# ChainSafe/co-zkvms

Measured on AMD Instinct MI355X. Metric: RISC-V cycles proved/sec (co-Jolt hot path: PST13 commit + dense GKR grand product + openings), higher is better.
Workload: dtype u32-limb BN254 Fr/Fq (254-bit Montgomery integers); 1 GPU; configs[1] restated (SURVEY 8d): 2^20-cycle trace per GPU, plain prover, 128 polys (64 Fr + 32 u16 + 16 u32 + 16 flags) PST13 batch commit, dense grand product 8 x 2^21 leaves, batch evaluate + opening reduction + PST13 open; log_n=20, polys=128, gp_batch=8, parallelism=single GPU, ranks_per_gpu=1

## Files before the change

co-zkvms_amd/csrc/msm.hip:

```cpp
#include "common.hpp"
#include "fq9.hip.hpp"

static constexpr uint32_t NB = 1u << 15;
static constexpr int CH = 16;
static constexpr int TPB = 256;

template <int KIND>
struct ScalarKind;
template <>
struct ScalarKind<COZK_SCALAR_FR> {
    static constexpr int NWIN = 16;
    static __device__ __forceinline__ bool load(const void* p, size_t i, uint32_t w[8]) {
        fe s = Fr::from_mont(fe_load(reinterpret_cast<const fe*>(p) + i));
#pragma unroll
        for (int k = 0; k < 8; k++) w[k] = s.l[k];
        return false;
    }
};
template <>
struct ScalarKind<COZK_SCALAR_U8> {
    static constexpr int NWIN = 1;
    static __device__ __forceinline__ bool load(const void* p, size_t i, uint32_t w[8]) {
        w[0] = reinterpret_cast<const uint8_t*>(p)[i];
        return false;
    }
};
template <>
struct ScalarKind<COZK_SCALAR_U16> {
    static constexpr int NWIN = 2;
    static __device__ __forceinline__ bool load(const void* p, size_t i, uint32_t w[8]) {
        w[0] = reinterpret_cast<const uint16_t*>(p)[i];
        return false;
    }
};
template <>
struct ScalarKind<COZK_SCALAR_U32> {
    static constexpr int NWIN = 3;
    static __device__ __forceinline__ bool load(const void* p, size_t i, uint32_t w[8]) {
        w[0] = reinterpret_cast<const uint32_t*>(p)[i];
        w[1] = 0;
        return false;
    }
};
template <>
struct ScalarKind<COZK_SCALAR_U64> {
    static constexpr int NWIN = 5;
    static __device__ __forceinline__ bool load(const void* p, size_t i, uint32_t w[8]) {
        uint64_t v = reinterpret_cast<const uint64_t*>(p)[i];
        w[0] = (uint32_t)v;
        w[1] = (uint32_t)(v >> 32);
        w[2] = 0;
        return false;
    }
};
template <>
struct ScalarKind<COZK_SCALAR_I64> {
    static constexpr int NWIN = 5;
    static __device__ __forceinline__ bool load(const void* p, size_t i, uint32_t w[8]) {
        int64_t v = reinterpret_cast<const int64_t*>(p)[i];
        bool neg = v < 0;
        uint64_t m = neg ? (uint64_t)0 - (uint64_t)v : (uint64_t)v;
        w[0] = (uint32_t)m;
        w[1] = (uint32_t)(m >> 32);
        w[2] = 0;
        return neg;
    }
};

static inline int kind_nwin(int kind) {
    switch (kind) {
        case COZK_SCALAR_FR: return 16;
        case COZK_SCALAR_U8: return 1;
        case COZK_SCALAR_U16: return 2;
        case COZK_SCALAR_U32: return 3;
        default: return 5;
    }
}

template <int KIND, class F>
__device__ __forceinline__ void for_each_digit(const void* scalars, size_t i, F&& f) {
    uint32_t w[8] = {0, 0, 0, 0, 0, 0, 0, 0};
    bool neg = ScalarKind<KIND>::load(scalars, i, w);
    uint32_t carry = 0;
#pragma unroll
    for (int k = 0; k < ScalarKind<KIND>::NWIN; k++) {
        uint32_t v = ((w[k >> 1] >> (16 * (k & 1))) & 0xffffu) + carry;
        bool sub = v > 32768u;
        carry = sub ? 1u : 0u;
        uint32_t mag = sub ? 65536u - v : v;
        f(k, mag, sub != neg);
    }
}

static __device__ __forceinline__ uint32_t agg_atomic_add(uint32_t* counters, uint32_t key, bool active) {
    uint64_t act = __ballot(active);
    uint32_t pos = 0;
    if (act == 0) return 0;
    int lane = threadIdx.x & 63;
    int first = __ffsll((unsigned long long)act) - 1;
    uint32_t k0 = __shfl(key, first);
    uint64_t same = __ballot(active && key == k0);
    int cnt = __popcll(same);
    bool merged = false;
    if (cnt >= 4) {
        uint32_t base = 0;
        if (lane == first) base = atomicAdd(&counters[k0], (uint32_t)cnt);
        base = __shfl(base, first);
        if (active && key == k0) {
            pos = base + __popcll(same & ((1ull << lane) - 1ull));
            merged = true;
        }
    }
    if (active && !merged) pos = atomicAdd(&counters[key], 1u);
    return pos;
}

template <int KIND>
__global__ void __launch_bounds__(TPB) k_msm_hist(const void* scalars, size_t n, uint32_t* hist, int grouped) {
    size_t i = (size_t)blockIdx.x * TPB + threadIdx.x;
    bool inr = i < n;
    size_t ii = inr ? i : 0;
    for_each_digit<KIND>(scalars, ii, [&](int k, uint32_t mag, bool) {
        bool act = inr && mag != 0;
        uint32_t key = (grouped ? (uint32_t)k * NB : 0u) + (mag - 1u);
        agg_atomic_add(hist, act ? key : 0u, act);
    });
}

template <int KIND>
__global__ void __launch_bounds__(TPB) k_msm_scatter(const void* scalars, size_t n, uint32_t* cursor, uint32_t* refs,
                                                  int grouped, uint32_t table_n, uint32_t base_off) {
    size_t i = (size_t)blockIdx.x * TPB + threadIdx.x;
    bool inr = i < n;
    size_t ii = inr ? i : 0;
    for_each_digit<KIND>(scalars, ii, [&](int k, uint32_t mag, bool negative) {
        bool act = inr && mag != 0;
        uint32_t key = (grouped ? (uint32_t)k * NB : 0u) + (mag - 1u);
        uint32_t pos = agg_atomic_add(cursor, act ? key : 0u, act);
        if (act) {
            uint32_t ref = (grouped ? 0u : (uint32_t)k * table_n) + base_off + (uint32_t)ii;
            refs[pos] = ref | (negative ? 0x80000000u : 0u);
        }
    });
}

struct MsmPolyDesc {
    const void* scalars;
    uint32_t n;
    uint32_t base_off;
    uint32_t group;
    uint32_t pad;
};
static constexpr int LTPB = 1024;

template <int KIND>
__global__ void __launch_bounds__(LTPB) k_msm_hist_lds(const MsmPolyDesc* __restrict__ descs, uint32_t* __restrict__ hist) {
    __shared__ uint32_t lh[NB];
    const MsmPolyDesc d = descs[blockIdx.y];
    for (uint32_t b = threadIdx.x; b < NB; b += blockDim.x) lh[b] = 0;
    __syncthreads();
    for (size_t i = (size_t)blockIdx.x * blockDim.x + threadIdx.x; i < d.n; i += (size_t)gridDim.x * blockDim.x) {
        for_each_digit<KIND>(d.scalars, i, [&](int, uint32_t mag, bool) {
            if (mag != 0) atomicAdd(&lh[mag - 1u], 1u);
        });
    }
    __syncthreads();
    uint32_t* h = hist + (size_t)d.group * NB;
    for (uint32_t b = threadIdx.x; b < NB; b += blockDim.x) {
        uint32_t c = lh[b];
        if (c) atomicAdd(&h[b], c);
    }
}

template <int KIND>
__global__ void __launch_bounds__(LTPB) k_msm_scatter_lds(const MsmPolyDesc* __restrict__ descs, uint32_t* __restrict__ cursor,
                                                       uint32_t* __restrict__ refs, uint32_t table_n) {
    __shared__ uint32_t lh[NB];
    const MsmPolyDesc d = descs[blockIdx.y];
    for (uint32_t b = threadIdx.x; b < NB; b += blockDim.x) lh[b] = 0;
    __syncthreads();
    for (size_t i = (size_t)blockIdx.x * blockDim.x + threadIdx.x; i < d.n; i += (size_t)gridDim.x * blockDim.x) {
        for_each_digit<KIND>(d.scalars, i, [&](int, uint32_t mag, bool) {
            if (mag != 0) atomicAdd(&lh[mag - 1u], 1u);
        });
    }
    __syncthreads();
    uint32_t* cur = cursor + (size_t)d.group * NB;
    for (uint32_t b = threadIdx.x; b < NB; b += blockDim.x) {
        uint32_t c = lh[b];
        lh[b] = c ? atomicAdd(&cur[b], c) : 0u;
    }
    __syncthreads();
    for (size_t i = (size_t)blockIdx.x * blockDim.x + threadIdx.x; i < d.n; i += (size_t)gridDim.x * blockDim.x) {
        for_each_digit<KIND>(d.scalars, i, [&](int k, uint32_t mag, bool negative) {
            if (mag != 0) {
                uint32_t pos = atomicAdd(&lh[mag - 1u], 1u);
                uint32_t ref = (uint32_t)k * table_n + d.base_off + (uint32_t)i;
                refs[pos] = ref | (negative ? 0x80000000u : 0u);
            }
        });
    }
}

static constexpr uint32_t SCAN_PER_BLOCK = 1024;

template <bool FROM_OFFSETS>
static __device__ __forceinline__ void scan_load4(const uint32_t* __restrict__ in, uint32_t nb, uint32_t L, uint32_t b0, uint32_t c[4],
                                                  const uint32_t* __restrict__ perm) {
#pragma unroll
    for (int k = 0; k < 4; k++) {
        uint32_t b = b0 + k;
        if (b >= nb) c[k] = 0;
        else if (FROM_OFFSETS) {
            uint32_t q = perm ? perm[b] : b;
            c[k] = (in[q + 1] - in[q] + L - 1u) / L;
        } else c[k] = in[b];
    }
}

static __device__ __forceinline__ uint32_t block_exclusive_scan_256(uint32_t v, uint32_t* sh4, uint32_t* total) {
    uint32_t x = v;
#pragma unroll
    for (int off = 1; off < 64; off <<= 1) {
        uint32_t y = __shfl_up(x, off);
        if ((int)(threadIdx.x & 63) >= off) x += y;
    }
    int w = threadIdx.x >> 6;
    if ((threadIdx.x & 63) == 63) sh4[w] = x;
    __syncthreads();
    uint32_t base = 0;
    for (int i = 0; i < w; i++) base += sh4[i];
    if (total) *total = sh4[0] + sh4[1] + sh4[2] + sh4[3];
    __syncthreads();
    return base + x - v;
}

template <bool FROM_OFFSETS>
__global__ void __launch_bounds__(256) k_scan_sums(const uint32_t* __restrict__ in, uint32_t nb, uint32_t L, uint32_t* __restrict__ bsums,
                                                 const uint32_t* __restrict__ perm) {
    __shared__ uint32_t sh4[4];
    uint32_t c[4];
    scan_load4<FROM_OFFSETS>(in, nb, L, blockIdx.x * SCAN_PER_BLOCK + threadIdx.x * 4, c, perm);
    uint32_t tot;
    (void)block_exclusive_scan_256(c[0] + c[1] + c[2] + c[3], sh4, &tot);
    if (threadIdx.x == 0) bsums[blockIdx.x] = tot;
}

__global__ void __launch_bounds__(1024) k_scan_top(uint32_t* bsums, uint32_t nblk, uint32_t* total_out) {
    __shared__ uint32_t sh[1024];
    uint32_t tid = threadIdx.x;
    uint32_t per = (nblk + 1023u) / 1024u;
    uint32_t b0 = tid * per, b1 = min(nblk, b0 + per);
    uint32_t sum = 0;
    for (uint32_t b = b0; b < b1; b++) sum += bsums[b];
    sh[tid] = sum;
    __syncthreads();
    for (uint32_t d = 1; d < 1024; d <<= 1) {
        uint32_t v = tid >= d ? sh[tid - d] : 0;
        __syncthreads();
        sh[tid] += v;
        __syncthreads();
    }
    uint32_t run = sh[tid] - sum;
    for (uint32_t b = b0; b < b1; b++) {
        uint32_t c = bsums[b];
        bsums[b] = run;
        run += c;
    }
    if (tid == 1023) *total_out = sh[1023];
}

template <bool FROM_OFFSETS>
__global__ void __launch_bounds__(256) k_scan_final(const uint32_t* in, uint32_t nb, uint32_t L, const uint32_t* __restrict__ bsums,
                                                  uint32_t* off, uint32_t* cursor, const uint32_t* __restrict__ perm) {
    __shared__ uint32_t sh4[4];
    uint32_t c[4];
    uint32_t b0 = blockIdx.x * SCAN_PER_BLOCK + threadIdx.x * 4;
    scan_load4<FROM_OFFSETS>(in, nb, L, b0, c, perm);
    uint32_t run = bsums[blockIdx.x] + block_exclusive_scan_256(c[0] + c[1] + c[2] + c[3], sh4, nullptr);
// ... 175 lines not shown
    xyzz9 acc;
    bool have = false;
    uint32_t ref_next = PF && begin < end ? refs[begin] : 0u;
    for (uint32_t e = begin; e < end; e++) {
        uint32_t ref = PF ? ref_next : refs[e];
        if (PF && e + 1 < end) ref_next = refs[e + 1];
        g1_affine p = affine_load(table + (ref & 0x7fffffffu));
        if (CHECK_INF && G1::is_inf(p)) continue;
        f9 qx = f9_from_fe(p.x), qy = f9_from_fe(p.y);
        if (ref >> 31) {
#pragma unroll
            for (int i = 0; i < 9; i++) qy.l[i] = F9_C2[i] - qy.l[i];
        }
        if (!have) {
            acc = xyzz9_from_affine(qx, qy);
            have = true;
        } else if (!madd9(acc, qx, qy)) {
            exc[1 + atomicAdd(exc, 1u)] = t;
            return;
        }
    }
    xyzz_store(out + slot, have ? xyzz9_to_xyzz(acc) : G1::identity());
}
__global__ void __launch_bounds__(TPB) k_msm_accum0_fix(const g1_affine* __restrict__ table, const uint32_t* __restrict__ refs,
                                                     const uint32_t* __restrict__ off_in, const uint32_t* __restrict__ off_out,
                                                     uint32_t nb, g1_xyzz* __restrict__ out, const uint32_t* __restrict__ exc,
                                                     const uint32_t* __restrict__ offp, const uint32_t* __restrict__ perm) {
    uint32_t n = exc[0];
    for (uint32_t q = blockIdx.x * TPB + threadIdx.x; q < n; q += gridDim.x * TPB) {
        uint32_t t = exc[1 + q];
        uint32_t begin, end, slot;
        segment_range_perm(off_in, off_out, offp, perm, nb, t, nullptr, begin, end, slot);
        xyzz_store(out + slot, gather_segment(table, refs, begin, end));
    }
}

__global__ void __launch_bounds__(TPB) k_msm_accumN(const g1_xyzz* __restrict__ in, const uint32_t* __restrict__ off_in,
                                                 const uint32_t* __restrict__ off_out, uint32_t nb, uint32_t L,
                                                 g1_xyzz* __restrict__ out, const uint32_t* __restrict__ blk) {
    uint32_t t = blockIdx.x * TPB + threadIdx.x;
    uint32_t total = off_out[nb];
    if (t >= total) return;
    uint32_t b = find_bucket_blk(off_out, nb, blk, t);
    uint32_t s = t - off_out[b];
    uint32_t cnt = off_in[b + 1] - off_in[b];
    uint32_t nseg = off_out[b + 1] - off_out[b];
    uint32_t per = (cnt + nseg - 1) / nseg;
    (void)L;
    uint32_t begin = off_in[b] + min(s * per, cnt);
    uint32_t end = off_in[b] + min((s + 1) * per, cnt);
    g1_xyzz acc = G1::identity();
    if (begin < end) acc = xyzz_load(in + begin);
    for (uint32_t e = begin + 1; e < end; e++) acc = G1::add(acc, xyzz_load(in + e));
    xyzz_store(out + t, acc);
}

static __device__ __forceinline__ g1_xyzz bucket_value(const g1_xyzz* items, const uint32_t* off, uint32_t b) {
    uint32_t o = off[b];
    if (off[b + 1] > o) return xyzz_load(items + o);
    return G1::identity();
}

__global__ void __launch_bounds__(TPB) k_msm_gather_buckets(const g1_xyzz* __restrict__ items, const uint32_t* __restrict__ off,
                                                         uint32_t nb, g1_xyzz* __restrict__ dense) {
    uint32_t b = blockIdx.x * TPB + threadIdx.x;
    if (b >= nb) return;
    xyzz_store(dense + b, bucket_value(items, off, b));
}

__global__ void __launch_bounds__(TPB) k_msm_reduce_chunks(const g1_xyzz* __restrict__ dense, uint32_t ngroups,
                                                        g1_xyzz* __restrict__ chunk_out) {
    uint32_t t = blockIdx.x * TPB + threadIdx.x;
    const uint32_t cpg = NB / CH;
    if (t >= ngroups * cpg) return;
    uint32_t g = t / cpg, c = t % cpg;
    uint32_t k0 = c * CH;
    g1_xyzz run = G1::identity(), acc = G1::identity();
    for (int j = CH - 1; j >= 0; j--) {
        run = G1::add(run, xyzz_load(dense + (size_t)g * NB + k0 + (uint32_t)j));
        acc = G1::add(acc, run);
    }
    if (c != 0 && !G1::is_identity(run)) {
        g1_xyzz m = G1::identity();
        for (int bit = 10; bit >= 0; bit--) {
            m = G1::dbl(m);
            if ((c >> bit) & 1u) m = G1::add(m, run);
        }
        for (int d = 0; d < 4; d++) m = G1::dbl(m);
        acc = G1::add(acc, m);
    }
    xyzz_store(chunk_out + t, acc);
}

__global__ void __launch_bounds__(TPB) k_msm_reduce_groups(const g1_xyzz* __restrict__ chunk, g1_xyzz* __restrict__ grp) {
    __shared__ g1_xyzz sh[TPB];
    const uint32_t cpg = NB / CH;
    uint32_t g = blockIdx.x, tid = threadIdx.x;
    g1_xyzz acc = G1::identity();
    for (uint32_t c = tid; c < cpg; c += TPB) acc = G1::add(acc, xyzz_load(chunk + (size_t)g * cpg + c));
    sh[tid] = acc;
    __syncthreads();
    for (uint32_t s = TPB / 2; s > 0; s >>= 1) {
        if (tid < s) {
            acc = G1::add(acc, sh[tid + s]);
            sh[tid] = acc;
        }
        __syncthreads();
    }
    if (tid == 0) xyzz_store(grp + g, acc);
}

__global__ void k_msm_finalize(const g1_xyzz* __restrict__ grp, uint32_t G, uint32_t npoly, g1_affine* __restrict__ out) {
    uint32_t p = blockIdx.x * blockDim.x + threadIdx.x;
    if (p >= npoly) return;
    g1_xyzz acc = xyzz_load(grp + (size_t)p * G + (G - 1));
    for (int w = (int)G - 2; w >= 0; w--) {
        for (int d = 0; d < 16; d++) acc = G1::dbl(acc);
        acc = G1::add(acc, xyzz_load(grp + (size_t)p * G + w));
    }
    affine_store(out + p, G1::to_affine(acc));
}

__global__ void __launch_bounds__(TPB) k_precompute_window(const g1_affine* __restrict__ prev, g1_affine* __restrict__ next, size_t n) {
    size_t i = (size_t)blockIdx.x * TPB + threadIdx.x;
    if (i >= n) return;
    g1_xyzz acc = G1::dbl_affine(affine_load(prev + i));
    for (int d = 1; d < 16; d++) acc = G1::dbl(acc);
    affine_store(next + i, G1::to_affine(acc));
}

__global__ void __launch_bounds__(TPB) k_fixed_base_mul(const fe* __restrict__ scalars, g1_affine g, g1_affine* __restrict__ out, size_t n) {
    size_t i = (size_t)blockIdx.x * TPB + threadIdx.x;
    if (i >= n) return;
    fe s = Fr::from_mont(fe_load(scalars + i));
    g1_xyzz acc = G1::identity();
    for (int k = 7; k >= 0; k--) {
        uint32_t w = s.l[k];
        for (int b = 31; b >= 0; b--) {
            acc = G1::dbl(acc);
            if ((w >> b) & 1u) acc = G1::add_mixed(acc, g);
        }
    }
    affine_store(out + i, G1::to_affine(acc));
}

__global__ void __launch_bounds__(TPB) k_pair_sums(const g1_affine* __restrict__ in, g1_affine* __restrict__ out, size_t nout) {
    size_t i = (size_t)blockIdx.x * TPB + threadIdx.x;
    if (i >= nout) return;
    g1_xyzz acc = G1::from_affine(affine_load(in + 2 * i));
    acc = G1::add_mixed(acc, affine_load(in + 2 * i + 1));
    affine_store(out + i, G1::to_affine(acc));
}

static inline uint32_t cdiv(uint64_t a, uint64_t b) { return (uint32_t)((a + b - 1) / b); }

__global__ void __launch_bounds__(TPB) k_any_infinity(const g1_affine* __restrict__ pts, size_t n, uint32_t* __restrict__ flag) {
    size_t i = (size_t)blockIdx.x * TPB + threadIdx.x;
    if (i < n && G1::is_inf(affine_load(pts + i))) atomicOr(flag, 1u);
}
static void build_window_table(cozk_ctx* ctx, cozk_bases* b) {
    for (int w = 1; w < b->nwin; w++) {
        k_precompute_window<<<cdiv(b->n, TPB), TPB, 0, ctx->stream>>>(b->table + (size_t)(w - 1) * b->n,
                                                                     b->table + (size_t)w * b->n, b->n);
    }
    HIP_TRY(hipGetLastError());
    ctx->scratch.reserve(64);
    uint32_t* flag = ctx->scratch.as<uint32_t>();
    HIP_TRY(hipMemsetAsync(flag, 0, 4, ctx->stream));
    k_any_infinity<<<cdiv(b->n, TPB), TPB, 0, ctx->stream>>>(b->table, b->n, flag);
    uint32_t h = 1;
    HIP_TRY(hipMemcpyAsync(&h, flag, 4, hipMemcpyDeviceToHost, ctx->stream));
    HIP_TRY(hipStreamSynchronize(ctx->stream));
    b->has_inf = h != 0;
}

#define KIND_DISPATCH(kind, CALL)                                              \
    switch (kind) {                                                            \
        case COZK_SCALAR_FR: { constexpr int K = COZK_SCALAR_FR; CALL; } break;   \
        case COZK_SCALAR_U8: { constexpr int K = COZK_SCALAR_U8; CALL; } break;   \
        case COZK_SCALAR_U16: { constexpr int K = COZK_SCALAR_U16; CALL; } break; \
        case COZK_SCALAR_U32: { constexpr int K = COZK_SCALAR_U32; CALL; } break; \
        case COZK_SCALAR_U64: { constexpr int K = COZK_SCALAR_U64; CALL; } break; \
        case COZK_SCALAR_I64: { constexpr int K = COZK_SCALAR_I64; CALL; } break; \
        default: throw CozkError(COZK_ERR_INVALID_ARG, "unknown scalar kind");    \
    }

struct MsmSetPlan {
    uint32_t P = 0, G = 1, nb = 0, L0 = 8;
    uint64_t M = 0, bound = 0, maxseg0 = 0;
    bool pre = false;
};

static MsmSetPlan msm_plan(const cozk_bases* bases, const size_t* offsets, const size_t* ns, const int* kinds, size_t P) {
    COZK_REQUIRE(P >= 1, "msm: empty batch");
    COZK_REQUIRE((uint64_t)bases->n * (uint64_t)bases->nwin < (1ull << 31), "msm: table too large for 31-bit refs");
    MsmSetPlan pl;
    pl.P = (uint32_t)P;
    pl.pre = bases->nwin == 16;
    pl.G = pl.pre ? 1u : 16u;
    pl.nb = (uint32_t)P * pl.G * NB;
    for (size_t p = 0; p < P; p++) {
        COZK_REQUIRE(offsets[p] + ns[p] <= bases->n, "msm: base slice out of range");
        uint64_t m = (uint64_t)ns[p] * kind_nwin(kinds[p]);
        pl.M += m;
        if (m > pl.bound) pl.bound = m;
    }
    COZK_REQUIRE(pl.M < (1ull << 32), "msm: batch too large (reference count exceeds 32 bits)");
    uint32_t L0 = (uint32_t)(pl.M >> 18);
    if (L0 < 8) L0 = 8;
    if (L0 > 127) L0 = 127;
    pl.L0 = L0;
    pl.maxseg0 = pl.M / L0 + pl.nb;
    return pl;
}

static void msm_scan(hipStream_t st, uint32_t* bsums, uint32_t nb, bool from_offsets, const uint32_t* in, uint32_t L, uint32_t* off, uint32_t* cursor,
                     const uint32_t* perm = nullptr) {
    const uint32_t nscan_blocks = (nb + SCAN_PER_BLOCK - 1) / SCAN_PER_BLOCK;
    if (from_offsets) {
        k_scan_sums<true><<<nscan_blocks, 256, 0, st>>>(in, nb, L, bsums, perm);
        k_scan_top<<<1, 1024, 0, st>>>(bsums, nscan_blocks, off + nb);
        k_scan_final<true><<<nscan_blocks, 256, 0, st>>>(in, nb, L, bsums, off, cursor, perm);
    } else {
        k_scan_sums<false><<<nscan_blocks, 256, 0, st>>>(in, nb, L, bsums, nullptr);
        k_scan_top<<<1, 1024, 0, st>>>(bsums, nscan_blocks, off + nb);
        k_scan_final<false><<<nscan_blocks, 256, 0, st>>>(in, nb, L, bsums, off, cursor, nullptr);
    }
}

static void msm_sort(cozk_ctx* ctx, hipStream_t st, MsmSortWs& sw, const MsmSetPlan& pl, const cozk_bases* bases, const size_t* offsets,
                     const size_t* ns, const void* const* scalars, const int* kinds) {
    const uint32_t nb = pl.nb, G = pl.G;
    const size_t P = pl.P;
    sw.hist.reserve((size_t)(nb + 2) * 4);
    sw.off0.reserve((size_t)(nb + 1) * 4);
    sw.offA.reserve((size_t)(nb + 1) * 4);
    sw.refs.reserve((size_t)pl.M * 4);
    uint32_t* hist = sw.hist.as<uint32_t>();
    uint32_t* off0 = sw.off0.as<uint32_t>();
    uint32_t* refs = sw.refs.as<uint32_t>();
    const uint32_t nscan_blocks = (nb + SCAN_PER_BLOCK - 1) / SCAN_PER_BLOCK;
    sw.ptrs.reserve((size_t)nscan_blocks * 4 + P * sizeof(MsmPolyDesc) + 64);
    uint32_t* bsums = sw.ptrs.as<uint32_t>();
    MsmPolyDesc* d_descs = reinterpret_cast<MsmPolyDesc*>(((uintptr_t)(bsums + nscan_blocks) + 15) & ~(uintptr_t)15);
    HIP_TRY(hipMemsetAsync(hist, 0, (size_t)(nb + 2) * 4, st));
    uint32_t* d_maxcnt = hist + nb + 1;
    if (!sw.max_pinned) HIP_TRY(hipHostMalloc((void**)&sw.max_pinned, 64 + 64 * sizeof(MsmPolyDesc), hipHostMallocDefault));
    if (!sw.max_event) HIP_TRY(hipEventCreateWithFlags(&sw.max_event, hipEventDisableTiming));
    auto read_back_max = [&] {
        k_max_u32<<<std::min<uint32_t>(cdiv(nb, 256), 1024u), 256, 0, st>>>(hist, nb, d_maxcnt);
        HIP_TRY(hipMemcpyAsync(sw.max_pinned, d_maxcnt, 4, hipMemcpyDeviceToHost, st));
        HIP_TRY(hipEventRecord(sw.max_event, st));
    };
    if (pl.pre) {
        MsmPolyDesc* h_descs = reinterpret_cast<MsmPolyDesc*>(reinterpret_cast<char*>(sw.max_pinned) + 64);
        COZK_REQUIRE(P <= 64, "msm: too many polynomials in one launch set");
        uint32_t nd = 0;
        std::vector<std::pair<int, std::pair<uint32_t, uint32_t>>> runs;
        size_t max_n = 0;
        for (int kind = 0; kind <= COZK_SCALAR_I64; kind++) {
            uint32_t first = nd;
            for (size_t p = 0; p < P; p++)
                if (kinds[p] == kind && ns[p]) {
                    h_descs[nd++] = MsmPolyDesc{scalars[p], (uint32_t)ns[p], (uint32_t)offsets[p], (uint32_t)p, 0};
                    if (ns[p] > max_n) max_n = ns[p];
                }
            if (nd > first) runs.push_back({kind, {first, nd - first}});
        }
        HIP_TRY(hipMemcpyAsync(d_descs, h_descs, nd * sizeof(MsmPolyDesc), hipMemcpyHostToDevice, st));
        static const int ltpb = getenv("COZK_MSM_LTPB") ? atoi(getenv("COZK_MSM_LTPB")) : 256;
        static const uint32_t wgs_max = getenv("COZK_MSM_WGS") ? (uint32_t)atoi(getenv("COZK_MSM_WGS")) : 64u;
        COZK_REQUIRE(ltpb >= 64 && ltpb <= LTPB && ltpb % 64 == 0, "COZK_MSM_LTPB out of range");
        COZK_REQUIRE(wgs_max >= 1 && wgs_max <= 1024, "COZK_MSM_WGS out of range (1..1024)");
        uint32_t wgs = (uint32_t)((max_n + 4095) / 4096);
        if (wgs < 1) wgs = 1;
        if (wgs > wgs_max) wgs = wgs_max;
        for (auto& r : runs) {
            dim3 grid(wgs, r.second.second);
            KIND_DISPATCH(r.first, (k_msm_hist_lds<K><<<grid, ltpb, 0, st>>>(d_descs + r.second.first, hist)));
        }
        read_back_max();
        msm_scan(st, bsums, nb, false, hist, 1, off0, hist);
        for (auto& r : runs) {
            dim3 grid(wgs, r.second.second);
            uint64_t alg = 0;
            for (uint32_t q = 0; q < r.second.second; q++) {
                const MsmPolyDesc& d = h_descs[r.second.first + q];
                const uint64_t sb = scalar_kind_bytes(r.first);
                alg += (uint64_t)d.n * (sb + 4ull * ((sb * 8 + 15) / 16));
            }
            ProfScope prof(ctx, COZK_PROF_MSM_SCATTER, alg, st);
            KIND_DISPATCH(r.first, (k_msm_scatter_lds<K><<<grid, ltpb, 0, st>>>(d_descs + r.second.first, hist, refs, (uint32_t)bases->n)));
        }
    } else {
        for (size_t p = 0; p < P; p++) {
            uint32_t* h = hist + (size_t)p * G * NB;
            if (ns[p]) KIND_DISPATCH(kinds[p], (k_msm_hist<K><<<cdiv(ns[p], TPB), TPB, 0, st>>>(scalars[p], ns[p], h, 1)));
        }
        read_back_max();
        msm_scan(st, bsums, nb, false, hist, 1, off0, hist);
        for (size_t p = 0; p < P; p++) {
            uint32_t* cur = hist + (size_t)p * G * NB;
            if (ns[p])
                KIND_DISPATCH(kinds[p], (k_msm_scatter<K><<<cdiv(ns[p], TPB), TPB, 0, st>>>(scalars[p], ns[p], cur, refs, 1, (uint32_t)bases->n,
                                                                                         (uint32_t)offsets[p])));
        }
    }
    msm_scan(st, bsums, nb, true, off0, pl.L0, sw.offA.as<uint32_t>(), nullptr);
    HIP_TRY(hipGetLastError());
}

static void msm_accumulate(cozk_ctx* ctx, MsmSortWs& sw, const MsmSetPlan& pl, const cozk_bases* bases, const size_t* ns, const int* kinds,
                           g1_xyzz* dense_out) {
    MsmWorkspace& ws = ctx->msm_ws;
    hipStream_t st = ctx->stream;
    const uint32_t nb = pl.nb, L0 = pl.L0;
    const uint32_t L1 = 8;
    const uint64_t maxseg0 = pl.maxseg0;
    const uint64_t maxpart = maxseg0 > 2ull * nb ? maxseg0 : 2ull * nb;
    ws.partA.reserve((size_t)maxpart * sizeof(g1_xyzz));
    ws.partB.reserve((size_t)maxpart * sizeof(g1_xyzz));
    ws.offB.reserve((size_t)(nb + 1) * 4);
    ws.offC.reserve((size_t)(nb + 1) * 4);
    ws.ptrs.reserve((size_t)((nb + SCAN_PER_BLOCK - 1) / SCAN_PER_BLOCK) * 4 + 64);
    uint32_t* refs = sw.refs.as<uint32_t>();
    uint32_t* off0 = sw.off0.as<uint32_t>();
    uint32_t* offA = sw.offA.as<uint32_t>();
    hipEvent_t e0 = nullptr, e1 = nullptr;
    if (ctx->prof_enabled) {
        HIP_TRY(hipEventCreate(&e0));
        HIP_TRY(hipEventCreate(&e1));
        HIP_TRY(hipEventRecord(e0, st));
    }
    ws.blk.reserve((size_t)(cdiv(maxpart, TPB) + 2) * 4);
    uint32_t* blk = ws.blk.as<uint32_t>();
    if (pl.pre) {
        ws.exc.reserve((size_t)(maxseg0 + 2) * 4);
        uint32_t* exc = ws.exc.as<uint32_t>();
        HIP_TRY(hipMemsetAsync(exc, 0, 4, st));
        ws.perm.reserve((size_t)nb * 4);
        ws.offP.reserve((size_t)(nb + 1) * 4 + SEGKEYS * 4);
        uint32_t* perm = ws.perm.as<uint32_t>();
        uint32_t* offP = ws.offP.as<uint32_t>();
        uint32_t* bins = offP + nb + 1;
        HIP_TRY(hipMemsetAsync(bins, 0, SEGKEYS * 4, st));
        k_seg_hist<<<cdiv(nb, 1024), 1024, 0, st>>>(off0, offA, nb, bins);
        k_seg_bins<<<1, 1, 0, st>>>(bins);
        k_seg_perm<<<cdiv(nb, 1024), 1024, 0, st>>>(off0, offA, nb, bins, perm);
        msm_scan(st, ws.ptrs.as<uint32_t>(), nb, true, offA, 1, offP, nullptr, perm);
        const uint32_t nblk0 = cdiv(maxseg0, TPB);
        k_block_buckets<<<cdiv(nblk0 + 1, 256), 256, 0, st>>>(offP, nb, nblk0, blk);
        if (bases->has_inf)
            k_msm_accum0_f9<true><<<nblk0, TPB, 0, st>>>(bases->table, refs, off0, offA, nb, ws.partA.as<g1_xyzz>(), exc, blk, offP, perm);
        else
            k_msm_accum0_f9<false, true><<<nblk0, TPB, 0, st>>>(bases->table, refs, off0, offA, nb, ws.partA.as<g1_xyzz>(), exc, blk, offP, perm);
        k_msm_accum0_fix<<<256, TPB, 0, st>>>(bases->table, refs, off0, offA, nb, ws.partA.as<g1_xyzz>(), exc, offP, perm);
    } else {
        k_msm_accum0<<<cdiv(maxseg0, TPB), TPB, 0, st>>>(bases->table, refs, off0, offA, nb, L0, ws.partA.as<g1_xyzz>());
    }
    if (ctx->prof_enabled) {
        HIP_TRY(hipEventRecord(e1, st));
        ctx->prof_events.push_back({e0, e1});
        ctx->prof_launches += 1;
        ctx->prof_units += pl.M;
        for (size_t p = 0; p < pl.P; p++) ctx->prof_alg_bytes += (uint64_t)ns[p] * (64 + scalar_kind_bytes(kinds[p]));
    }
    HIP_TRY(hipEventSynchronize(sw.max_event));
    uint64_t fullest = *(volatile uint32_t*)sw.max_pinned;
    COZK_REQUIRE(fullest <= pl.bound, "msm: histogram larger than the reference count");
    uint64_t cnt = (fullest + L0 - 1) / L0;
    uint64_t maxseg = maxseg0;
    g1_xyzz* cur_items = ws.partA.as<g1_xyzz>();
    g1_xyzz* nxt_items = ws.partB.as<g1_xyzz>();
    uint32_t* cur_off = offA;
    uint32_t* nxt_off = ws.offB.as<uint32_t>();
    uint32_t* spare_off = ws.offC.as<uint32_t>();
    while (cnt > 1) {
        uint64_t nseg = maxseg / L1 + nb;
        msm_scan(st, ws.ptrs.as<uint32_t>(), nb, true, cur_off, L1, nxt_off, nullptr);
        const uint32_t nblkN = cdiv(nseg, TPB);
        k_block_buckets<<<cdiv(nblkN + 1, 256), 256, 0, st>>>(nxt_off, nb, nblkN, blk);
        k_msm_accumN<<<nblkN, TPB, 0, st>>>(cur_items, cur_off, nxt_off, nb, L1, nxt_items, blk);
        std::swap(cur_items, nxt_items);
        uint32_t* done = cur_off;
        cur_off = nxt_off;
        nxt_off = (done == offA) ? spare_off : done;
        maxseg = nseg;
        cnt = (cnt + L1 - 1) / L1;
    }
    k_msm_gather_buckets<<<cdiv(nb, TPB), TPB, 0, st>>>(cur_items, cur_off, nb, dense_out);
    HIP_TRY(hipGetLastError());
}

static void affine_to_abi(const g1_affine& a, uint64_t xy[8], int* inf) {
    bool is_inf = G1::is_inf(a);
    for (int i = 0; i < 4; i++) {
        xy[i] = (uint64_t)a.x.l[2 * i] | ((uint64_t)a.x.l[2 * i + 1] << 32);
        xy[4 + i] = (uint64_t)a.y.l[2 * i] | ((uint64_t)a.y.l[2 * i + 1] << 32);
    }
    if (inf) *inf = is_inf ? 1 : 0;
}
static g1_affine abi_to_affine(const uint64_t xy[8], int inf) {
    g1_affine a;
    for (int i = 0; i < 4; i++) {
        a.x.l[2 * i] = (uint32_t)xy[i];
        a.x.l[2 * i + 1] = (uint32_t)(xy[i] >> 32);
        a.y.l[2 * i] = (uint32_t)xy[4 + i];
        a.y.l[2 * i + 1] = (uint32_t)(xy[4 + i] >> 32);
    }
    if (inf) {
        a.x = Fq::zero();
        a.y = Fq::zero();
    }
    return a;
}

void msm_batch(cozk_ctx* ctx, const cozk_bases* bases, const size_t* offsets, const size_t* ns, const void* const* scalars,
               const int* kinds, size_t k, uint64_t* out_xy, int* out_inf) {
    MsmWorkspace& ws = ctx->msm_ws;
    hipStream_t st = ctx->stream;
    const uint32_t G = bases->nwin == 16 ? 1u : 16u;
    const size_t maxP = bases->nwin == 16 ? 64 : 4;
    const size_t tail_cap = 256 / G;
    ws.out.reserve(k * sizeof(g1_affine));
    g1_affine* d_out = ws.out.as<g1_affine>();
    for (size_t t0 = 0; t0 < k; t0 += tail_cap) {
        size_t kt = k - t0 < tail_cap ? k - t0 : tail_cap;
        const uint32_t ngroups = (uint32_t)kt * G;
        ws.bsum.reserve((size_t)ngroups * NB * sizeof(g1_xyzz));
        ws.chunk.reserve((size_t)ngroups * (NB / CH) * sizeof(g1_xyzz));
        ws.grp.reserve((size_t)ngroups * sizeof(g1_xyzz));
        g1_xyzz* dense = ws.bsum.as<g1_xyzz>();
        struct SetRange { size_t s, P; };
        std::vector<SetRange> sets;
        uint64_t set_refs_cap;
        {
            static const int pinned = getenv("COZK_MSM_SET_REFS_LOG2") ? atoi(getenv("COZK_MSM_SET_REFS_LOG2")) : 0;
            if (pinned) set_refs_cap = 1ull << (pinned < 24 ? 24 : (pinned > 31 ? 31 : pinned));
            else {
                uint64_t total = 0;
                for (size_t p = 0; p < kt; p++) total += (uint64_t)ns[t0 + p] * kind_nwin(kinds[t0 + p]);
                set_refs_cap = total / 4;
                if (set_refs_cap < (1ull << 28)) set_refs_cap = 1ull << 28;
                if (set_refs_cap > (1ull << 30)) set_refs_cap = 1ull << 30;
            }
        }
        {
            size_t s = 0;
            while (s < kt) {
                size_t P = 0;
                uint64_t M = 0;
                while (s + P < kt && P < maxP) {
                    uint64_t m = (uint64_t)ns[t0 + s + P] * kind_nwin(kinds[t0 + s + P]);
                    if (P > 0 && M + m > set_refs_cap) break;
                    M += m;
                    P++;
                }
                sets.push_back({s, P});
                s += P;
            }
        }
        if (sets.size() > 2) {
            size_t best = 0;
            uint64_t best_m = ~0ull;
            for (size_t i = 0; i < sets.size(); i++) {
                uint64_t m = 0;
                for (size_t p = 0; p < sets[i].P; p++) m += (uint64_t)ns[t0 + sets[i].s + p] * kind_nwin(kinds[t0 + sets[i].s + p]);
                if (m < best_m) {
                    best_m = m;
                    best = i;
                }
            }
            std::rotate(sets.begin(), sets.begin() + best, sets.begin() + best + 1);
        }
        static const bool pipeline = getenv("COZK_MSM_SERIAL") == nullptr;
        hipStream_t side = st;
        if (pipeline && sets.size() > 1) {
            if (!ctx->stream2) {
                static const bool prio = getenv("COZK_MSM_NO_PRIORITY") == nullptr;
                int lo = 0, hi = 0;
                HIP_TRY(hipDeviceGetStreamPriorityRange(&lo, &hi));
                if (prio) HIP_TRY(hipStreamCreateWithPriority(&ctx->stream2, hipStreamNonBlocking, hi));
                else HIP_TRY(hipStreamCreateWithFlags(&ctx->stream2, hipStreamNonBlocking));
            }
            side = ctx->stream2;
        }
        for (int b = 0; b < 2; b++) {
            if (!ws.sort[b].done) HIP_TRY(hipEventCreateWithFlags(&ws.sort[b].done, hipEventDisableTiming));
            if (!ws.sort[b].consumed) HIP_TRY(hipEventCreateWithFlags(&ws.sort[b].consumed, hipEventDisableTiming));
        }
        if (side != st) {
            if (!ws.fork) HIP_TRY(hipEventCreateWithFlags(&ws.fork, hipEventDisableTiming));
            HIP_TRY(hipEventRecord(ws.fork, st));
            HIP_TRY(hipStreamWaitEvent(side, ws.fork, 0));
        }
        std::vector<MsmSetPlan> plans(sets.size());
        auto launch_sort = [&](size_t i) {
            const SetRange& r = sets[i];
            plans[i] = msm_plan(bases, offsets + t0 + r.s, ns + t0 + r.s, kinds + t0 + r.s, r.P);
            if (plans[i].M == 0) return;
            MsmSortWs& sw = ws.sort[i & 1];
            if (i >= 2 && side != st) HIP_TRY(hipStreamWaitEvent(side, sw.consumed, 0));
            msm_sort(ctx, side, sw, plans[i], bases, offsets + t0 + r.s, ns + t0 + r.s, scalars + t0 + r.s, kinds + t0 + r.s);
            if (side != st) HIP_TRY(hipEventRecord(sw.done, side));
        };
        if (!sets.empty()) launch_sort(0);
        for (size_t i = 0; i < sets.size(); i++) {
            if (side != st && i + 1 < sets.size()) launch_sort(i + 1);
            const SetRange& r = sets[i];
            g1_xyzz* out_i = dense + (size_t)r.s * G * NB;
            if (plans[i].M != 0) {
                MsmSortWs& sw = ws.sort[i & 1];
                if (side != st) HIP_TRY(hipStreamWaitEvent(st, sw.done, 0));
                msm_accumulate(ctx, sw, plans[i], bases, ns + t0 + r.s, kinds + t0 + r.s, out_i);
                if (side != st) HIP_TRY(hipEventRecord(sw.consumed, st));
            } else {
                HIP_TRY(hipMemsetAsync(out_i, 0, (size_t)plans[i].nb * sizeof(g1_xyzz), st));
            }
            if (side == st && i + 1 < sets.size()) launch_sort(i + 1);
        }
        k_msm_reduce_chunks<<<cdiv((uint64_t)ngroups * (NB / CH), TPB), TPB, 0, st>>>(dense, ngroups, ws.chunk.as<g1_xyzz>());
        k_msm_reduce_groups<<<ngroups, TPB, 0, st>>>(ws.chunk.as<g1_xyzz>(), ws.grp.as<g1_xyzz>());
        k_msm_finalize<<<cdiv(kt, 64), 64, 0, st>>>(ws.grp.as<g1_xyzz>(), G, (uint32_t)kt, d_out + t0);
        HIP_TRY(hipGetLastError());
    }
    g1_affine* h = reinterpret_cast<g1_affine*>(ctx_pinned(ctx, k * sizeof(g1_affine)));
    HIP_TRY(hipMemcpyAsync(h, d_out, k * sizeof(g1_affine), hipMemcpyDeviceToHost, st));
    HIP_TRY(hipStreamSynchronize(st));
    for (size_t i = 0; i < k; i++) affine_to_abi(h[i], out_xy + 8 * i, out_inf ? out_inf + i : nullptr);
}

extern "C" {

int cozk_bases_upload(cozk_ctx* ctx, const uint64_t* xy, const uint8_t* infinity, size_t n, int precompute,
                      cozk_bases** out) {
    return cozk_guard(ctx, [&] {
        COZK_REQUIRE(ctx && xy && out && n > 0, "bases_upload: bad argument");
        cozk_bases* b = new cozk_bases{ctx, n, precompute ? 16 : 1, nullptr};
        try {
            HIP_TRY(hipMalloc((void**)&b->table, (size_t)b->nwin * n * sizeof(g1_affine)));
            std::vector<g1_affine> h(n);
            for (size_t i = 0; i < n; i++) h[i] = abi_to_affine(xy + 8 * i, infinity ? infinity[i] : 0);
            HIP_TRY(hipMemcpyAsync(b->table, h.data(), n * sizeof(g1_affine), hipMemcpyHostToDevice, ctx->stream));
            HIP_TRY(hipStreamSynchronize(ctx->stream));
            build_window_table(ctx, b);
            HIP_TRY(hipStreamSynchronize(ctx->stream));
        } catch (...) {
            if (b->table) (void)hipFree(b->table);
            delete b;
            throw;
        }
        *out = b;
    });
}

int cozk_bases_from_scalars(cozk_ctx* ctx, const cozk_vec* s, const uint64_t* g_xy, int precompute, cozk_bases** out) {
    return cozk_guard(ctx, [&] {
        COZK_REQUIRE(ctx && s && g_xy && out && s->kind == COZK_SCALAR_FR && s->n > 0, "bases_from_scalars: bad argument");
        size_t n = s->n;
        cozk_bases* b = new cozk_bases{ctx, n, precompute ? 16 : 1, nullptr};
        try {
            HIP_TRY(hipMalloc((void**)&b->table, (size_t)b->nwin * n * sizeof(g1_affine)));
            g1_affine g = abi_to_affine(g_xy, 0);
            k_fixed_base_mul<<<cdiv(n, TPB), TPB, 0, ctx->stream>>>(reinterpret_cast<const fe*>(s->d), g, b->table, n);
            HIP_TRY(hipGetLastError());
            build_window_table(ctx, b);
            HIP_TRY(hipStreamSynchronize(ctx->stream));
        } catch (...) {
            if (b->table) (void)hipFree(b->table);
            delete b;
            throw;
        }
        *out = b;
    });
}

int cozk_bases_pair_sums(cozk_ctx* ctx, const cozk_bases* src, int precompute, cozk_bases** out) {
    return cozk_guard(ctx, [&] {
        COZK_REQUIRE(ctx && src && out && src->n >= 2 && src->n % 2 == 0, "bases_pair_sums: bad argument");
        size_t n = src->n / 2;
        cozk_bases* b = new cozk_bases{ctx, n, precompute ? 16 : 1, nullptr};
        try {
            HIP_TRY(hipMalloc((void**)&b->table, (size_t)b->nwin * n * sizeof(g1_affine)));
            k_pair_sums<<<cdiv(n, TPB), TPB, 0, ctx->stream>>>(src->table, b->table, n);
            HIP_TRY(hipGetLastError());
            build_window_table(ctx, b);
            HIP_TRY(hipStreamSynchronize(ctx->stream));
        } catch (...) {
            if (b->table) (void)hipFree(b->table);
            delete b;
            throw;
        }
        *out = b;
    });
}

int cozk_bases_download(cozk_ctx* ctx, const cozk_bases* b, size_t offset, size_t n, uint64_t* xy, uint8_t* infinity) {
    return cozk_guard(ctx, [&] {
        COZK_REQUIRE(ctx && b && xy && offset + n <= b->n, "bases_download: bad argument");
        std::vector<g1_affine> h(n);
        HIP_TRY(hipMemcpyAsync(h.data(), b->table + offset, n * sizeof(g1_affine), hipMemcpyDeviceToHost, ctx->stream));
        HIP_TRY(hipStreamSynchronize(ctx->stream));
        for (size_t i = 0; i < n; i++) {
            int inf;
            affine_to_abi(h[i], xy + 8 * i, &inf);
            if (infinity) infinity[i] = (uint8_t)inf;
        }
    });
}

int cozk_bases_free(cozk_bases* b) {
    if (!b) return COZK_OK;
    if (b->table) (void)hipFree(b->table);
    delete b;
    return COZK_OK;
}

size_t cozk_bases_len(const cozk_bases* b) { return b ? b->n : 0; }

int cozk_msm_vec(cozk_ctx* ctx, const cozk_bases* bases, size_t offset, const cozk_vec* scalars, uint64_t out_xy[8],
                 int* out_infinity) {
    return cozk_guard(ctx, [&] {
        COZK_REQUIRE(ctx && bases && scalars && out_xy, "msm_vec: bad argument");
        const void* p = scalars->d;
        int kind = scalars->kind;
        size_t n = scalars->n;
        msm_batch(ctx, bases, &offset, &n, &p, &kind, 1, out_xy, out_infinity);
    });
}

int cozk_batch_msm_vec(cozk_ctx* ctx, const cozk_bases* bases, size_t offset, const cozk_vec* const* scalars, size_t k,
                       uint64_t* out_xy, int* out_infinity) {
    return cozk_guard(ctx, [&] {
        COZK_REQUIRE(ctx && bases && scalars && out_xy && k > 0, "batch_msm_vec: bad argument");
        std::vector<const void*> ptrs(k);
        std::vector<int> kinds(k);
        std::vector<size_t> offs(k, offset), ns(k);
        size_t n = scalars[0]->n;
        for (size_t i = 0; i < k; i++) {
            COZK_REQUIRE(scalars[i] && scalars[i]->n == n, "batch_msm_vec: polynomials must have equal length");
            ptrs[i] = scalars[i]->d;
            kinds[i] = scalars[i]->kind;
            ns[i] = n;
        }
        msm_batch(ctx, bases, offs.data(), ns.data(), ptrs.data(), kinds.data(), k, out_xy, out_infinity);
    });
}

int cozk_batch_msm_slices(cozk_ctx* ctx, const cozk_bases* bases, const size_t* offsets, const cozk_vec* const* scalars,
                          const size_t* lens, size_t k, uint64_t* out_xy, int* out_infinity) {
    return cozk_guard(ctx, [&] {
        COZK_REQUIRE(ctx && bases && offsets && scalars && out_xy && k > 0, "batch_msm_slices: bad argument");
        std::vector<const void*> ptrs(k);
        std::vector<int> kinds(k);
        std::vector<size_t> ns(k);
        for (size_t i = 0; i < k; i++) {
            COZK_REQUIRE(scalars[i], "batch_msm_slices: null scalar vector");
            ns[i] = lens ? lens[i] : scalars[i]->n;
            COZK_REQUIRE(ns[i] <= scalars[i]->n, "batch_msm_slices: length exceeds the scalar vector");
            ptrs[i] = scalars[i]->d;
            kinds[i] = scalars[i]->kind;
        }
        msm_batch(ctx, bases, offsets, ns.data(), ptrs.data(), kinds.data(), k, out_xy, out_infinity);
    });
// ... 102 lines not shown
```

Baseline: 9.114 million cycles/s.

## Widen MSM signed-digit windows from 16 to 17 bits

Switches the Pippenger MSM from 16-bit to 17-bit signed windows. Fr scalars now need 15 windows instead of 16, and small-integer kinds need one fewer window each, which cuts the number of bucket references and the window-table size. Bucket count per group doubles to 2^16, so the LDS histogram and scatter kernels each handle a 32K-bucket half selected by grid.z, and the chunk/group reduction and doubling counts are updated to match. In exchange, every scalar is read twice (once per half), and bucket reduction does more work per group.

```diff
diff --git a/co-zkvms_amd/csrc/msm.hip b/co-zkvms_amd/csrc/msm.hip
--- a/co-zkvms_amd/csrc/msm.hip
+++ b/co-zkvms_amd/csrc/msm.hip
@@ -1,15 +1,20 @@
 #include "common.hpp"
 #include "fq9.hip.hpp"
 
-static constexpr uint32_t NB = 1u << 15;
+static constexpr int C = 17;
+static constexpr int NWIN_FR = 15;
+static constexpr uint32_t NB = 1u << (C - 1);
 static constexpr int CH = 16;
+static constexpr int CPG_LOG2 = C - 1 - 4;
+static_assert(CH << CPG_LOG2 == (int)NB, "CH must be 2^4");
+static_assert(NWIN_FR * C >= 255, "15 signed 17-bit windows must cover an Fr scalar plus its carry");
 static constexpr int TPB = 256;
 
 template <int KIND>
 struct ScalarKind;
 template <>
 struct ScalarKind<COZK_SCALAR_FR> {
-    static constexpr int NWIN = 16;
+    static constexpr int NWIN = NWIN_FR;
     static __device__ __forceinline__ bool load(const void* p, size_t i, uint32_t w[8]) {
         fe s = Fr::from_mont(fe_load(reinterpret_cast<const fe*>(p) + i));
 #pragma unroll
@@ -27,7 +32,7 @@
 };
 template <>
 struct ScalarKind<COZK_SCALAR_U16> {
-    static constexpr int NWIN = 2;
+    static constexpr int NWIN = 1;
     static __device__ __forceinline__ bool load(const void* p, size_t i, uint32_t w[8]) {
         w[0] = reinterpret_cast<const uint16_t*>(p)[i];
         return false;
@@ -35,7 +40,7 @@
 };
 template <>
 struct ScalarKind<COZK_SCALAR_U32> {
-    static constexpr int NWIN = 3;
+    static constexpr int NWIN = 2;
     static __device__ __forceinline__ bool load(const void* p, size_t i, uint32_t w[8]) {
         w[0] = reinterpret_cast<const uint32_t*>(p)[i];
         w[1] = 0;
@@ -44,7 +49,7 @@
 };
 template <>
 struct ScalarKind<COZK_SCALAR_U64> {
-    static constexpr int NWIN = 5;
+    static constexpr int NWIN = 4;
     static __device__ __forceinline__ bool load(const void* p, size_t i, uint32_t w[8]) {
         uint64_t v = reinterpret_cast<const uint64_t*>(p)[i];
         w[0] = (uint32_t)v;
@@ -55,7 +60,7 @@
 };
 template <>
 struct ScalarKind<COZK_SCALAR_I64> {
-    static constexpr int NWIN = 5;
+    static constexpr int NWIN = 4;
     static __device__ __forceinline__ bool load(const void* p, size_t i, uint32_t w[8]) {
         int64_t v = reinterpret_cast<const int64_t*>(p)[i];
         bool neg = v < 0;
@@ -69,11 +74,11 @@
 
 static inline int kind_nwin(int kind) {
     switch (kind) {
-        case COZK_SCALAR_FR: return 16;
-        case COZK_SCALAR_U8: return 1;
-        case COZK_SCALAR_U16: return 2;
-        case COZK_SCALAR_U32: return 3;
-        default: return 5;
+        case COZK_SCALAR_FR: return ScalarKind<COZK_SCALAR_FR>::NWIN;
+        case COZK_SCALAR_U8: return ScalarKind<COZK_SCALAR_U8>::NWIN;
+        case COZK_SCALAR_U16: return ScalarKind<COZK_SCALAR_U16>::NWIN;
+        case COZK_SCALAR_U32: return ScalarKind<COZK_SCALAR_U32>::NWIN;
+        default: return ScalarKind<COZK_SCALAR_U64>::NWIN;
     }
 }
 
@@ -84,10 +89,13 @@
     uint32_t carry = 0;
 #pragma unroll
     for (int k = 0; k < ScalarKind<KIND>::NWIN; k++) {
-        uint32_t v = ((w[k >> 1] >> (16 * (k & 1))) & 0xffffu) + carry;
-        bool sub = v > 32768u;
+        const int bit = C * k, wd = bit >> 5, sh = bit & 31;
+        uint32_t raw = w[wd] >> sh;
+        if (sh + C > 32 && wd + 1 < 8) raw |= w[wd + 1] << (32 - sh);
+        uint32_t v = (raw & ((1u << C) - 1u)) + carry;
+        bool sub = v > NB;
         carry = sub ? 1u : 0u;
-        uint32_t mag = sub ? 65536u - v : v;
+        uint32_t mag = sub ? (1u << C) - v : v;
         f(k, mag, sub != neg);
     }
 }
@@ -152,21 +160,26 @@
     uint32_t pad;
 };
 static constexpr int LTPB = 1024;
+static constexpr uint32_t LDS_NB = 1u << 15;
+static constexpr uint32_t LDS_HALVES = NB / LDS_NB;
+static_assert(LDS_HALVES == 2, "the LDS sort splits a bucket group in two halves");
 
 template <int KIND>
 __global__ void __launch_bounds__(LTPB) k_msm_hist_lds(const MsmPolyDesc* __restrict__ descs, uint32_t* __restrict__ hist) {
-    __shared__ uint32_t lh[NB];
+    __shared__ uint32_t lh[LDS_NB];
     const MsmPolyDesc d = descs[blockIdx.y];
-    for (uint32_t b = threadIdx.x; b < NB; b += blockDim.x) lh[b] = 0;
+    const uint32_t half = blockIdx.z;
+    for (uint32_t b = threadIdx.x; b < LDS_NB; b += blockDim.x) lh[b] = 0;
     __syncthreads();
     for (size_t i = (size_t)blockIdx.x * blockDim.x + threadIdx.x; i < d.n; i += (size_t)gridDim.x * blockDim.x) {
         for_each_digit<KIND>(d.scalars, i, [&](int, uint32_t mag, bool) {
-            if (mag != 0) atomicAdd(&lh[mag - 1u], 1u);
+            uint32_t b = mag - 1u;
+            if (mag != 0 && b / LDS_NB == half) atomicAdd(&lh[b % LDS_NB], 1u);
         });
     }
     __syncthreads();
-    uint32_t* h = hist + (size_t)d.group * NB;
-    for (uint32_t b = threadIdx.x; b < NB; b += blockDim.x) {
+    uint32_t* h = hist + (size_t)d.group * NB + (size_t)half * LDS_NB;
+    for (uint32_t b = threadIdx.x; b < LDS_NB; b += blockDim.x) {
         uint32_t c = lh[b];
         if (c) atomicAdd(&h[b], c);
     }
@@ -175,26 +188,29 @@
 template <int KIND>
 __global__ void __launch_bounds__(LTPB) k_msm_scatter_lds(const MsmPolyDesc* __restrict__ descs, uint32_t* __restrict__ cursor,
                                                        uint32_t* __restrict__ refs, uint32_t table_n) {
-    __shared__ uint32_t lh[NB];
+    __shared__ uint32_t lh[LDS_NB];
     const MsmPolyDesc d = descs[blockIdx.y];
-    for (uint32_t b = threadIdx.x; b < NB; b += blockDim.x) lh[b] = 0;
+    const uint32_t half = blockIdx.z;
+    for (uint32_t b = threadIdx.x; b < LDS_NB; b += blockDim.x) lh[b] = 0;
     __syncthreads();
     for (size_t i = (size_t)blockIdx.x * blockDim.x + threadIdx.x; i < d.n; i += (size_t)gridDim.x * blockDim.x) {
         for_each_digit<KIND>(d.scalars, i, [&](int, uint32_t mag, bool) {
-            if (mag != 0) atomicAdd(&lh[mag - 1u], 1u);
+            uint32_t b = mag - 1u;
+            if (mag != 0 && b / LDS_NB == half) atomicAdd(&lh[b % LDS_NB], 1u);
         });
     }
     __syncthreads();
-    uint32_t* cur = cursor + (size_t)d.group * NB;
-    for (uint32_t b = threadIdx.x; b < NB; b += blockDim.x) {
+    uint32_t* cur = cursor + (size_t)d.group * NB + (size_t)half * LDS_NB;
+    for (uint32_t b = threadIdx.x; b < LDS_NB; b += blockDim.x) {
         uint32_t c = lh[b];
         lh[b] = c ? atomicAdd(&cur[b], c) : 0u;
     }
     __syncthreads();
     for (size_t i = (size_t)blockIdx.x * blockDim.x + threadIdx.x; i < d.n; i += (size_t)gridDim.x * blockDim.x) {
         for_each_digit<KIND>(d.scalars, i, [&](int k, uint32_t mag, bool negative) {
-            if (mag != 0) {
-                uint32_t pos = atomicAdd(&lh[mag - 1u], 1u);
+            uint32_t b = mag - 1u;
+            if (mag != 0 && b / LDS_NB == half) {
+                uint32_t pos = atomicAdd(&lh[b % LDS_NB], 1u);
                 uint32_t ref = (uint32_t)k * table_n + d.base_off + (uint32_t)i;
                 refs[pos] = ref | (negative ? 0x80000000u : 0u);
             }
@@ -536,7 +552,7 @@
     }
     if (c != 0 && !G1::is_identity(run)) {
         g1_xyzz m = G1::identity();
-        for (int bit = 10; bit >= 0; bit--) {
+        for (int bit = CPG_LOG2 - 1; bit >= 0; bit--) {
             m = G1::dbl(m);
             if ((c >> bit) & 1u) m = G1::add(m, run);
         }
@@ -569,7 +585,7 @@
     if (p >= npoly) return;
     g1_xyzz acc = xyzz_load(grp + (size_t)p * G + (G - 1));
     for (int w = (int)G - 2; w >= 0; w--) {
-        for (int d = 0; d < 16; d++) acc = G1::dbl(acc);
+        for (int d = 0; d < C; d++) acc = G1::dbl(acc);
         acc = G1::add(acc, xyzz_load(grp + (size_t)p * G + w));
     }
     affine_store(out + p, G1::to_affine(acc));
@@ -579,7 +595,7 @@
     size_t i = (size_t)blockIdx.x * TPB + threadIdx.x;
     if (i >= n) return;
     g1_xyzz acc = G1::dbl_affine(affine_load(prev + i));
-    for (int d = 1; d < 16; d++) acc = G1::dbl(acc);
+    for (int d = 1; d < C; d++) acc = G1::dbl(acc);
     affine_store(next + i, G1::to_affine(acc));
 }
 
@@ -650,8 +666,8 @@
     COZK_REQUIRE((uint64_t)bases->n * (uint64_t)bases->nwin < (1ull << 31), "msm: table too large for 31-bit refs");
     MsmSetPlan pl;
     pl.P = (uint32_t)P;
-    pl.pre = bases->nwin == 16;
-    pl.G = pl.pre ? 1u : 16u;
+    pl.pre = bases->nwin == NWIN_FR;
+    pl.G = pl.pre ? 1u : (uint32_t)NWIN_FR;
     pl.nb = (uint32_t)P * pl.G * NB;
     for (size_t p = 0; p < P; p++) {
         COZK_REQUIRE(offsets[p] + ns[p] <= bases->n, "msm: base slice out of range");
@@ -730,18 +746,17 @@
         if (wgs < 1) wgs = 1;
         if (wgs > wgs_max) wgs = wgs_max;
         for (auto& r : runs) {
-            dim3 grid(wgs, r.second.second);
+            dim3 grid(wgs, r.second.second, LDS_HALVES);
             KIND_DISPATCH(r.first, (k_msm_hist_lds<K><<<grid, ltpb, 0, st>>>(d_descs + r.second.first, hist)));
         }
         read_back_max();
         msm_scan(st, bsums, nb, false, hist, 1, off0, hist);
         for (auto& r : runs) {
-            dim3 grid(wgs, r.second.second);
+            dim3 grid(wgs, r.second.second, LDS_HALVES);
             uint64_t alg = 0;
             for (uint32_t q = 0; q < r.second.second; q++) {
                 const MsmPolyDesc& d = h_descs[r.second.first + q];
-                const uint64_t sb = scalar_kind_bytes(r.first);
-                alg += (uint64_t)d.n * (sb + 4ull * ((sb * 8 + 15) / 16));
+                alg += (uint64_t)d.n * (scalar_kind_bytes(r.first) + 4ull * kind_nwin(r.first));
             }
             ProfScope prof(ctx, COZK_PROF_MSM_SCATTER, alg, st);
             KIND_DISPATCH(r.first, (k_msm_scatter_lds<K><<<grid, ltpb, 0, st>>>(d_descs + r.second.first, hist, refs, (uint32_t)bases->n)));
@@ -873,8 +888,8 @@
                const int* kinds, size_t k, uint64_t* out_xy, int* out_inf) {
     MsmWorkspace& ws = ctx->msm_ws;
     hipStream_t st = ctx->stream;
-    const uint32_t G = bases->nwin == 16 ? 1u : 16u;
-    const size_t maxP = bases->nwin == 16 ? 64 : 4;
+    const uint32_t G = bases->nwin == NWIN_FR ? 1u : (uint32_t)NWIN_FR;
+    const size_t maxP = bases->nwin == NWIN_FR ? 64 : 4;
     const size_t tail_cap = 256 / G;
     ws.out.reserve(k * sizeof(g1_affine));
     g1_affine* d_out = ws.out.as<g1_affine>();
@@ -990,7 +1005,7 @@
                       cozk_bases** out) {
     return cozk_guard(ctx, [&] {
         COZK_REQUIRE(ctx && xy && out && n > 0, "bases_upload: bad argument");
-        cozk_bases* b = new cozk_bases{ctx, n, precompute ? 16 : 1, nullptr};
+        cozk_bases* b = new cozk_bases{ctx, n, precompute ? NWIN_FR : 1, nullptr};
         try {
             HIP_TRY(hipMalloc((void**)&b->table, (size_t)b->nwin * n * sizeof(g1_affine)));
             std::vector<g1_affine> h(n);
@@ -1012,7 +1027,7 @@
     return cozk_guard(ctx, [&] {
         COZK_REQUIRE(ctx && s && g_xy && out && s->kind == COZK_SCALAR_FR && s->n > 0, "bases_from_scalars: bad argument");
         size_t n = s->n;
-        cozk_bases* b = new cozk_bases{ctx, n, precompute ? 16 : 1, nullptr};
+        cozk_bases* b = new cozk_bases{ctx, n, precompute ? NWIN_FR : 1, nullptr};
         try {
             HIP_TRY(hipMalloc((void**)&b->table, (size_t)b->nwin * n * sizeof(g1_affine)));
             g1_affine g = abi_to_affine(g_xy, 0);
@@ -1033,7 +1048,7 @@
     return cozk_guard(ctx, [&] {
         COZK_REQUIRE(ctx && src && out && src->n >= 2 && src->n % 2 == 0, "bases_pair_sums: bad argument");
         size_t n = src->n / 2;
-        cozk_bases* b = new cozk_bases{ctx, n, precompute ? 16 : 1, nullptr};
+        cozk_bases* b = new cozk_bases{ctx, n, precompute ? NWIN_FR : 1, nullptr};
         try {
             HIP_TRY(hipMalloc((void**)&b->table, (size_t)b->nwin * n * sizeof(g1_affine)));
             k_pair_sums<<<cdiv(n, TPB), TPB, 0, ctx->stream>>>(src->table, b->table, n);
```

Result: slower. 8.566 million cycles/s (median of 2 runs) (-6.0%).
